# manoskary/analysisgnn

Measured on AMD Instinct MI355X. Metric: subgraph-nodes/sec fwd+bwd, HybridGNN L=3 H=256, higher is better.
Workload: dtype f32; 1 GPU; C2 (sampled, the batch a training step sees): HybridGNN L=3 H=256 out=128, 21 task heads, 32 neighbour-sampled subgraphs x (500 target notes + [5,5] hops) per GPU, per-hop counts passed (every layer trimmed); 16335 notes, 104099 edges per GPU; train step = fwd + objective (wloss) + bwd + allreduce + clip + AdamW, CSR rebuilt every step; hipGraph replay; workload_id=c2s, per_gpu_subgraphs=32, objective=wloss, parallelism=dp1, allreduce=none (one rank)

## Files before the change

analysisgnn_amd/_lib.py:

```python
from __future__ import annotations

import ctypes as C
import os
from typing import Optional, Sequence

import torch

from . import resident

_HERE = os.path.dirname(os.path.abspath(__file__))
LIB_PATH = os.path.join(_HERE, "libagnn_hip.so")
MAX_SEG = 32

SPMM_MEAN, SPMM_SKIP_SELF, SPMM_ACCUM = 1, 2, 4
INT32_MAX = 2 ** 31 - 1


class AgnnError(RuntimeError):
    pass


class CooSeg(C.Structure):
    _fields_ = [("row", C.c_void_p), ("col", C.c_void_p), ("etype", C.c_void_p),
                ("etype_code", C.c_int64), ("n_edges", C.c_int64), ("n_rows", C.c_int64)]
# ... 171 lines not shown
    "agnn_norm_act_fwd_f32": (C.c_int, [C.c_void_p, C.c_int64, C.c_void_p, C.c_void_p, C.c_int32, C.c_int64, C.c_int32, C.c_float, C.c_float,
                                        C.c_uint32, C.c_void_p, C.c_uint32, C.c_void_p, C.c_int64, C.c_void_p, C.c_void_p, C.c_void_p,
                                        C.c_void_p]),
    "agnn_norm_act_bwd_f32": (C.c_int, [C.c_void_p, C.c_int64, C.c_void_p, C.c_void_p, C.c_int32, C.c_int64, C.c_int32, C.c_float, C.c_float,
                                        C.c_uint32, C.c_void_p, C.c_uint32, C.c_void_p, C.c_int64, C.c_void_p, C.c_void_p, C.c_void_p,
                                        C.c_int64, C.c_void_p, C.c_void_p, C.c_void_p, C.c_size_t, C.c_void_p]),
    "agnn_norm_act_colsum_batch_f32": (C.c_int, [C.c_int32, C.POINTER(ColsumItem), C.c_void_p]),
    "agnn_skip_act_workspace_bytes": (C.c_size_t, []),
    "agnn_skip_act_fwd_f32": (C.c_int, [C.c_void_p, C.c_int64, C.c_void_p, C.c_int64, C.c_void_p, C.c_int64, C.c_int32, C.c_float, C.c_uint32,
                                        C.c_void_p, C.c_uint32, C.c_void_p, C.c_int64, C.c_void_p, C.c_void_p]),
    "agnn_skip_act_bwd_f32": (C.c_int, [C.c_void_p, C.c_int64, C.c_void_p, C.c_int64, C.c_void_p, C.c_int64, C.c_int32, C.c_float, C.c_uint32,
                                        C.c_void_p, C.c_uint32, C.c_void_p, C.c_int64, C.c_void_p, C.c_int64, C.c_void_p, C.c_int64, C.c_void_p,
                                        C.c_void_p, C.c_size_t, C.c_void_p]),
    "agnn_norm_act_colsum_f32": (C.c_int, [C.c_void_p, C.c_size_t, C.c_int64, C.c_int32, C.c_void_p, C.c_void_p, C.c_void_p]),
    "agnn_wgrad_workspace_bytes": (C.c_size_t, [C.c_int64, C.c_int32, C.c_int32]),
    "agnn_wgrad_f32": (C.c_int, [C.c_void_p, C.c_int64, C.c_void_p, C.c_int64, C.c_int64, C.c_int32, C.c_int32, C.c_void_p,
                                 C.c_int64, C.c_void_p, C.c_void_p, C.c_size_t, C.c_void_p]),
    "agnn_pack_f32": (C.c_int, [C.c_int32, C.POINTER(PackItem), C.c_void_p]),
    "agnn_gather_f32": (C.c_int, [C.c_int32, C.POINTER(GatherItem), C.c_void_p]),
    "agnn_debug_stamp": (C.c_int, [C.c_void_p, C.c_void_p]),
    "agnn_gproj_fwd_f32": (C.c_int, [C.c_void_p, C.c_int64, C.c_void_p, C.c_void_p, C.c_void_p, C.c_int32, C.c_int32, C.c_int32,
                                     C.c_int64, C.c_void_p, C.c_int64, C.c_void_p]),
    "agnn_gproj_workspace_bytes": (C.c_size_t, [C.c_int64, C.c_int32, C.c_int32, C.c_int32]),
    "agnn_gproj_bwd_f32": (C.c_int, [C.c_void_p, C.c_int64, C.c_void_p, C.c_int64, C.c_void_p, C.c_void_p, C.c_int32, C.c_int32,
                                     C.c_int32, C.c_int32, C.c_int64, C.c_void_p, C.c_int64, C.c_void_p, C.c_void_p, C.c_void_p,
                                     C.c_size_t, C.c_void_p]),
    "agnn_spmm_self_grad_f32": (C.c_int, [C.c_void_p, C.c_int64, C.c_int64, C.c_int32, C.c_void_p, C.c_int64, C.c_int64, C.c_int32,
                                          C.c_void_p, C.c_int64, C.c_int32, C.c_void_p]),
    "agnn_embed_cat_fwd_f32": (C.c_int, [C.c_void_p, C.c_int64, C.c_int32, C.c_int64, C.c_int32, C.POINTER(C.c_void_p),
                                         C.POINTER(C.c_void_p), C.POINTER(C.c_int32), C.c_int32, C.c_void_p, C.c_int64, C.c_void_p]),
    "agnn_embed_workspace_bytes": (C.c_size_t, [C.c_int32, C.POINTER(C.c_int32), C.c_int32]),
    "agnn_embed_cat_bwd_f32": (C.c_int, [C.c_void_p, C.c_int64, C.c_int32, C.c_int64, C.c_int32, C.POINTER(C.c_void_p),
                                         C.POINTER(C.c_int32), C.c_int32, C.c_void_p, C.c_void_p, C.c_size_t, C.c_void_p]),
    "agnn_train_loss_workspace_bytes": (C.c_size_t, []),
    "agnn_train_loss_f32": (C.c_int, [C.c_void_p, C.c_int64, C.c_void_p, C.c_int32, C.c_void_p, C.c_int64, C.c_float, C.c_int64,
                                      C.c_void_p, C.c_int64, C.c_int32, C.c_float, C.c_void_p, C.c_float, C.c_void_p, C.c_void_p,
                                      C.c_void_p, C.c_void_p, C.c_void_p, C.c_void_p, C.c_void_p, C.c_void_p, C.c_size_t,
                                      C.c_void_p]),
    "agnn_train_loss_final_f32": (C.c_int, [C.c_void_p, C.c_int64, C.c_void_p, C.c_int32, C.c_void_p, C.c_int64, C.c_float, C.c_int64,
                                            C.c_void_p, C.c_int64, C.c_int32, C.c_float, C.c_void_p, C.c_float, C.c_void_p, C.c_void_p,
                                            C.c_void_p, C.c_void_p, C.c_void_p, C.c_void_p, C.c_void_p, C.c_void_p, C.c_int64, C.c_void_p,
                                            C.c_size_t, C.c_void_p]),
    "agnn_train_loss_bwd_f32": (C.c_int, [C.c_void_p, C.c_int64, C.c_void_p, C.c_int32, C.c_int64, C.c_int32, C.c_void_p, C.c_void_p,
                                          C.c_void_p, C.c_int64, C.c_void_p, C.c_int64, C.c_int32, C.c_float, C.c_void_p, C.c_int64,
                                          C.c_void_p]),
    "agnn_adamw_workspace_bytes": (C.c_size_t, []),
    "agnn_adamw_f32": (C.c_int, [C.c_void_p, C.c_void_p, C.c_void_p, C.c_void_p, C.c_int64, C.c_float, C.c_float, C.c_float,
                                 C.c_float, C.c_float, C.c_float, C.c_void_p, C.c_void_p, C.c_int32, C.c_void_p, C.c_size_t,
                                 C.c_void_p]),
    "agnn_lr_schedule_at": (C.c_double, [C.POINTER(LrSchedule), C.c_int64]),
    "agnn_adamw_sched_workspace_bytes": (C.c_size_t, []),
    "agnn_adamw_sched_f32": (C.c_int, [C.c_void_p, C.c_void_p, C.c_void_p, C.c_void_p, C.c_int64, C.POINTER(LrSchedule), C.c_float,
                                       C.c_float, C.c_float, C.c_float, C.c_float, C.c_void_p, C.c_void_p, C.c_void_p, C.c_void_p,
                                       C.c_int32, C.c_void_p, C.c_size_t, C.c_void_p]),
    "agnn_multitask_ce_f32": (C.c_int, [C.c_void_p, C.c_int64, C.c_void_p, C.c_int32, C.c_void_p, C.c_int64, C.c_float,
                                        C.c_int64, C.c_void_p, C.c_void_p, C.c_void_p, C.c_void_p, C.c_void_p]),
    "agnn_multitask_ce_scale_f32": (C.c_int, [C.c_void_p, C.c_int64, C.c_void_p, C.c_int32, C.c_int64, C.c_int32, C.c_void_p,
                                              C.c_void_p, C.c_int64, C.c_void_p]),
    "agnn_kd_workspace_bytes": (C.c_size_t, [C.c_int64, C.c_int32]),
    "agnn_multitask_kd_f32": (C.c_int, [C.c_void_p, C.c_int64, C.c_void_p, C.c_int64, C.c_void_p, C.c_void_p, C.c_int32, C.c_int64,
                                        C.c_int32, C.c_float, C.c_float, C.c_void_p, C.c_int64, C.c_void_p, C.c_void_p, C.c_void_p,
                                        C.c_size_t, C.c_void_p]),
    "agnn_ewc_workspace_bytes": (C.c_size_t, []),
    "agnn_ewc_f32": (C.c_int, [C.c_void_p, C.c_void_p, C.c_void_p, C.c_int64, C.c_float, C.c_void_p, C.c_void_p, C.c_void_p,
                               C.c_size_t, C.c_void_p]),
    "agnn_fisher_accum_f32": (C.c_int, [C.c_void_p, C.c_int64, C.c_float, C.c_void_p, C.c_void_p]),
# ... 99 lines not shown
```

analysisgnn_amd/csrc/embed.hip:

```cpp
#include <cstdlib>

#include "agnn_common.h"

namespace {

constexpr int kMaxTab = AGNN_EMBED_MAX_TABLES;
constexpr int kSlices = 128;

struct EmbFwd {
  const float* x;
  int64_t ld_x;
  int32_t in_x, n_tab, dim;
  int64_t n_rows;
  const int64_t* idx[kMaxTab];
  const float* tab[kMaxTab];
  int32_t vocab[kMaxTab];
  float* out;
  int64_t ld_out;
};

__global__ __launch_bounds__(256) void k_embed_cat_fwd(EmbFwd a) {
  const int64_t total = a.n_rows * a.ld_out;
  for (int64_t e = static_cast<int64_t>(blockIdx.x) * 256 + threadIdx.x; e < total; e += static_cast<int64_t>(gridDim.x) * 256) {
    const int64_t row = e / a.ld_out;
// ... 152 lines not shown
  if (n_tab <= 0 || n_tab > kMaxTab) return fail(AGNN_EINVAL, "embed_bwd: n_tab=%d not in [1,%d]", n_tab, kMaxTab);
  if (n_rows < 0 || col0 < 0 || dim <= 0 || (dim & 1)) return fail(AGNN_EINVAL, "embed_bwd: bad sizes n_rows=%lld col0=%d dim=%d (dim must be even)", (long long)n_rows, col0, dim);
  if (!dout || !idx || !vocab || !dtables || !workspace) return fail(AGNN_EINVAL, "embed_bwd: null argument");
  if (ld_dout < static_cast<int64_t>(col0) + static_cast<int64_t>(n_tab) * dim) return fail(AGNN_EINVAL, "embed_bwd: ld_dout smaller than the row");
  if (reinterpret_cast<uintptr_t>(dtables) & 7u) return fail(AGNN_EALIGN, "embed_bwd: dtables must be 8-byte aligned");
  const size_t need = agnn_embed_workspace_bytes(n_tab, vocab, dim);
  if (need == 0 || workspace_bytes < need) return fail(AGNN_ENOMEM, "embed_bwd: workspace %zu < %zu bytes", workspace_bytes, need);
  EmbBwd a{};
  a.dout = dout; a.ld_dout = ld_dout; a.col0 = col0; a.n_tab = n_tab; a.dim = dim; a.dim_pad = dim; a.n_rows = n_rows;
  int vt = 0;
  for (int t = 0; t < n_tab; ++t) {
    if (!idx[t] || vocab[t] <= 0) return fail(AGNN_EINVAL, "embed_bwd: table %d: null index pointer or empty table", t);
    a.idx[t] = idx[t];
    a.vbase[t] = vt;
    vt += vocab[t];
  }
  a.vbase[n_tab] = vt;
  a.v_total = vt; a.v_pad = vt;
  a.slab = reinterpret_cast<float*>((reinterpret_cast<uintptr_t>(workspace) + 255) & ~uintptr_t{255});
  hipStream_t s = static_cast<hipStream_t>(stream_);
  const int ncg = (n_tab * dim + 63) / 64;
  if (static_cast<int64_t>(vt) * dim <= kEmbLdsFloats && ncg <= 4) {
    if (ncg == 1) hipLaunchKernelGGL(k_embed_bwd_rows<1>, dim3(kSlices), dim3(256), 0, s, a);
    else if (ncg == 2) hipLaunchKernelGGL(k_embed_bwd_rows<2>, dim3(kSlices), dim3(256), 0, s, a);
    else if (ncg == 3) hipLaunchKernelGGL(k_embed_bwd_rows<3>, dim3(kSlices), dim3(256), 0, s, a);
    else hipLaunchKernelGGL(k_embed_bwd_rows<4>, dim3(kSlices), dim3(256), 0, s, a);
    if (int rc = check_launch("embed_bwd(rows)")) return rc;
  } else {
    hipLaunchKernelGGL(k_embed_bwd, dim3(vt, kSlices), dim3(256), 0, s, a);
    if (int rc = check_launch("embed_bwd")) return rc;
  }
  return launch_slab_reduce(a.slab, nullptr, kSlices * 4, vt, dim, vt, dim, dtables, dim, nullptr, s);
}
```

analysisgnn_amd/embedding.py:

```python
from __future__ import annotations

import torch
import torch.nn.functional as F

import ctypes as C
from typing import Sequence

from . import _lib
from .linear import all_steal, weight_grad, wgrad_stream

MAX_ROWS = 256


class _SmallEmbedding(torch.autograd.Function):
    @staticmethod
    def forward(ctx, idx, weight):
        ctx.save_for_backward(idx)
        ctx.rows = weight.shape[0]
        ctx.leaf = weight.is_leaf
        ctx.weight_ref = weight if weight.is_leaf else None
        return F.embedding(idx, weight)

    @staticmethod
    def backward(ctx, dy):
        (idx,) = ctx.saved_tensors
        V = ctx.rows
        Vp = V + (V & 1)
        with wgrad_stream(dy.device, dy, idx, active=ctx.leaf and all_steal((ctx.weight_ref,)), kind="embed"):
            flat_idx = idx.reshape(-1)
            onehot = (flat_idx.unsqueeze(1) == torch.arange(Vp, device=idx.device)).to(dy.dtype)
            dy2 = dy.reshape(-1, dy.shape[-1]).contiguous()
            dw, _ = weight_grad(onehot, dy2, False)
            dw = dw[:V]
        return None, dw


def embedding(idx: torch.Tensor, weight: torch.Tensor) -> torch.Tensor:
    if weight.is_cuda and weight.requires_grad and torch.is_grad_enabled() and weight.shape[0] <= MAX_ROWS:
        return _SmallEmbedding.apply(idx, weight)
    return F.embedding(idx, weight)

# ... 26 lines not shown
        ctx.meta = (n, in_x, n_tab, dim, [int(t.shape[0]) for t in tabs], all(t.is_leaf for t in tabs))
        ctx.tab_refs = [t for t in tabs if t.is_leaf]
        return out[:, :width]

    @staticmethod
    def backward(ctx, dout):
        idc = ctx.saved_tensors
        n, in_x, n_tab, dim, vocabs, leaf = ctx.meta
        lib = _lib.load()
        dev = dout.device
        if dout.stride(1) != 1 or dout.dtype != torch.float32:
            dout = dout.float().contiguous()
        with wgrad_stream(dev, dout, *idc, active=leaf and all_steal(ctx.tab_refs), kind="embed"):
            vocab = (C.c_int32 * n_tab)(*vocabs)
            dtab = torch.empty((sum(vocabs), dim), dtype=torch.float32, device=dev)
            nws = int(lib.agnn_embed_workspace_bytes(n_tab, vocab, dim))
            ws = torch.empty(nws, dtype=torch.uint8, device=dev)
            _lib.check(lib.agnn_embed_cat_bwd_f32(dout.data_ptr(), dout.stride(0), in_x, n, n_tab, _ptr_array(idc), vocab, dim,
                                                  dtab.data_ptr(), ws.data_ptr(), nws, _lib.stream_ptr(dev)), "agnn_embed_cat_bwd_f32")
            grads = list(torch.split(dtab, vocabs, dim=0))
        return (None, None, *([None] * n_tab), *grads)


def embed_cat(x: torch.Tensor, idxs: Sequence[torch.Tensor], tables: Sequence[torch.Tensor]) -> torch.Tensor:
    n_tab = len(tables)
    fits = (x.is_cuda and x.dim() == 2 and 1 <= n_tab <= MAX_TABLES and len(idxs) == n_tab and not x.requires_grad
            and all(t.dim() == 2 and t.shape[1] == tables[0].shape[1] and t.dtype == torch.float32 for t in tables)
            and tables[0].shape[1] % 2 == 0 and all(i.dim() == 1 and i.shape[0] == x.shape[0] for i in idxs))
    if not fits:
        return torch.cat([x] + [embedding(i, t) for i, t in zip(idxs, tables)], dim=-1)
    r = _EmbedCat.apply(x, n_tab, *idxs, *tables)
    r._agnn_grad_cols = (int(x.shape[1]), int(r.shape[1]))
    return r
```

analysisgnn_amd/fused.py:

```python
from __future__ import annotations

import itertools
from typing import Optional

import torch
import torch.nn as nn
import torch.nn.functional as F

from . import _lib, resident
from .linear import ColsumItem, all_steal, defer, deferring, grad_slot_groups, leaf_refs, slot_group

PRE_RELU, POST_RELU = 1, 2
ENABLED = True
_CALL_IDS = itertools.count(1)


def rng_state(device) -> torch.Tensor:
    return resident.value(device, ("dropout counter",), lambda: torch.tensor([int(torch.initial_seed()) & 0x7FFFFFFFFFFFFFFF, 0],
                                                                             dtype=torch.int64, device=device))


def advance_rng(device) -> None:
    rng_state(device)[1:2].add_(1)

# ... 138 lines not shown
            raise _lib.AgnnError("norm_act: precomputed results stand for a plain LayerNorm on the kernel path")
        if not (torch.is_grad_enabled() and (x.requires_grad or ln.weight.requires_grad or ln.bias.requires_grad)):
            return pre[0]
        return _NormAct.apply(x, ln.weight, ln.bias, ln.eps, 0.0, 0, next(_CALL_IDS) & 0xFFFFFFFF, 0, False, None, pre)
    if not usable:
        y = F.relu(x) if pre_relu else x
        y = ln(y)
        y = F.relu(y) if post_relu else y
        return F.dropout(y, p, training)
    x2 = x.reshape(-1, H)
    flags = (PRE_RELU if pre_relu else 0) | (POST_RELU if post_relu else 0)
    y = _NormAct.apply(x2, ln.weight, ln.bias, ln.eps, p if training else 0.0, flags, next(_CALL_IDS) & 0xFFFFFFFF)
    return y.view(x.shape)


def grouped_norm_act(x: torch.Tensor, gamma: torch.Tensor, beta: torch.Tensor, eps: float, pre_relu: bool = False, pre=None) -> torch.Tensor:
    N, G, H = x.shape
    W = G * H
    gl = H // 4
    ok = (ENABLED and x.is_cuda and x.dtype == torch.float32 and H % 4 == 0 and 256 % H == 0 and (gl & (gl - 1)) == 0 and W <= 2048)
    if not ok:
        if pre is not None:
            raise _lib.AgnnError("grouped_norm_act: precomputed results need the kernel path")
        y = F.relu(x) if pre_relu else x
        return F.layer_norm(y, (H,), None, None, eps) * gamma + beta
    view_only = all(t.is_leaf or getattr(t, "_agnn_wgrad_deferrable", False) for t in (gamma, beta))
    y = _NormAct.apply(x.reshape(N, W), gamma.reshape(W), beta.reshape(W), eps, 0.0, PRE_RELU if pre_relu else 0,
                       next(_CALL_IDS) & 0xFFFFFFFF, H, view_only, leaf_refs(gamma, beta), pre, (slot_group(gamma), slot_group(beta)))
    return y.view(N, G, H)


class FusedSequential(nn.Sequential):

    def forward(self, x, pre=None):
        mods = list(self)
        i = 0
        if pre is not None:
            if not mods or not isinstance(mods[0], nn.LayerNorm) or (len(mods) > 1 and isinstance(mods[1], (nn.ReLU, nn.Dropout))):
                raise _lib.AgnnError("FusedSequential: precomputed results need a leading plain LayerNorm")
            x = norm_act(x, mods[0], pre=pre)
            i = 1
        while i < len(mods):
            m = mods[i]
            nxt = mods[i + 1] if i + 1 < len(mods) else None
            nn2 = mods[i + 2] if i + 2 < len(mods) else None
            if isinstance(m, nn.ReLU) and isinstance(nxt, nn.LayerNorm):
                p, used = (nn2.p, 3) if isinstance(nn2, nn.Dropout) else (0.0, 2)
                x = norm_act(x, nxt, pre_relu=True, p=p, training=self.training)
                i += used
            elif isinstance(m, nn.LayerNorm):
                post = isinstance(nxt, nn.ReLU)
                d = mods[i + 1 + int(post)] if i + 1 + int(post) < len(mods) else None
                p = d.p if isinstance(d, nn.Dropout) else 0.0
                x = norm_act(x, m, post_relu=post, p=p, training=self.training)
                i += 1 + int(post) + int(isinstance(d, nn.Dropout))
            else:
                x = m(x)
                i += 1
        return x
```

analysisgnn_amd/models.py:

```python
from __future__ import annotations

from typing import Dict, Optional

import torch
import torch.nn as nn
import torch.nn.functional as F

from . import _lib, ops
from .encoders import HybridGNN, MetricalGNN
from .fused import FusedSequential, _al16, advance_rng
from .embedding import embed_cat
from .heads import CrossTaskTransformer, fused_head_logits, fused_logit_fusion
from .linear import Linear
from .graph import SegSpec, build_csr


JOIN_FUSED = True


def _onset_index(n: int, onset_edges: torch.Tensor, batch_size: int, index):
    et = ("note", "onset", "note")
    if index is not None and et in index.bwd and index.bwd[et].n_rows >= n:
        return index.bwd[et], index.fwd[et]
    fwd, bwd = build_csr([SegSpec(onset_edges[0], onset_edges[1], n_rows=max(n, batch_size)),
                          SegSpec(onset_edges[1], onset_edges[0], n_rows=max(n, batch_size))])
    return fwd, bwd


class _PoolCat(torch.autograd.Function):

    @staticmethod
    def forward(ctx, x, fwd, bwd, n_pool, col_limit, gamma, beta, eps, box):
        dev = x.device
        lib = _lib.load()
        n, H = x.shape
        u = torch.empty((n, 2 * H), dtype=torch.float32, device=dev)
        y = torch.empty((n, 2 * H), dtype=torch.float32, device=dev)
        mean = torch.empty((n,), dtype=torch.float32, device=dev)
        rstd = torch.empty((n,), dtype=torch.float32, device=dev)
        inv_cnt = torch.empty((n,), dtype=torch.float32, device=dev)
        rel = _lib.make_rels([dict(src=None, rowptr=fwd.rowptr.data_ptr(), col=fwd.col.data_ptr(), ld_src=0)])
        _lib.check(lib.agnn_pool_cat_norm_f32(rel, x.data_ptr(), x.stride(0), n, n_pool, H, min(int(col_limit), _lib.INT32_MAX), gamma.data_ptr(),
                                              beta.data_ptr(), float(eps), u.data_ptr(), u.stride(0), y.data_ptr(), y.stride(0), mean.data_ptr(),
                                              rstd.data_ptr(), inv_cnt.data_ptr(), _lib.stream_ptr(dev)), "agnn_pool_cat_norm_f32")
        box.extend([y, mean, rstd])
        ctx.bwd, ctx.n_pool = bwd, n_pool
        ctx.save_for_backward(inv_cnt)
        return u

# ... 79 lines not shown
            self.cross_task_transformer = CrossTaskTransformer(o // 2, num_heads=4, dropout=dropout)
            self.fusion_layers = nn.ModuleDict({t: nn.Linear(o // 2, c) for t, c in task_dict.items()})
        self.rnn, self.rnn_norm, self.rnn_mlp = nn.Identity(), nn.Identity(), nn.Identity()

    def adjacent_parameter_groups(self):
        mods = list(self.clf_dict.values())
        groups = [[m[0].weight for m in mods], [m[0].bias for m in mods], [m[2].weight for m in mods],
                  [m[2].bias for m in mods], [m[3].weight for m in mods], [m[3].bias for m in mods]]
        rnn = getattr(self.encoder, "rnn", None)
        if isinstance(rnn, nn.GRU) and rnn.bidirectional:
            for layer in range(rnn.num_layers):
                for n in ("weight_ih", "weight_hh", "bias_ih", "bias_hh"):
                    groups.append([getattr(rnn, f"{n}_l{layer}"), getattr(rnn, f"{n}_l{layer}_reverse")])
        return groups

    split_backward = False

    def late_parameters(self):
        return [*self.project_dict.parameters(), *self.pitch_embedding.parameters(), *self.key_embedding.parameters()]

    def finish_backward(self) -> None:
        cut, self._cut = getattr(self, "_cut", None), None
        if cut:
            live = [(h, leaf.grad) for h, leaf in cut if leaf.grad is not None]
            if live:
                torch.autograd.backward([h for h, _ in live], [g for _, g in live])

    @torch._dynamo.disable
    def encode(self, pitch_spelling, key_signature, x_dict, edge_index_dict, batch_dict, batch_size,
               neighbor_mask_node, neighbor_mask_edge):
        if self.training:
            advance_rng(x_dict["note"].device)
        z_dict = dict(x_dict)
        z_dict["note"] = embed_cat(z_dict["note"], [pitch_spelling, key_signature],
                                   [self.pitch_embedding.weight, self.key_embedding.weight])
        for k, z in z_dict.items():
            if k != "note" and z.is_cuda and z.dim() == 2 and (z.shape[1] & 1) and z.stride(1) == 1 and z.stride(0) == z.shape[1] and z.shape[0] > 0:
                z_dict[k] = F.pad(z, (0, 1))[:, :z.shape[1]]
        h_dict = {k: self.project_dict[k](z_dict[k]) for k in self.project_dict.keys()}
        self._cut = None
        if self.split_backward and torch.is_grad_enabled():
            self._cut = []
            for k, hk in list(h_dict.items()):
                if hk.requires_grad:
                    leaf = hk.detach().requires_grad_(True)
                    self._cut.append((hk, leaf))
                    h_dict[k] = leaf
        x = self.encoder(x_dict=h_dict, edge_index_dict=edge_index_dict, batch_dict=batch_dict,
                         batch_size=batch_size, neighbor_mask_node=neighbor_mask_node,
                         neighbor_mask_edge=neighbor_mask_edge, return_edge_index=False, edge_attr_dict=None)
        index = getattr(getattr(self.encoder, "gnn", None), "last_index", None)
        onset = edge_index_dict[("note", "onset", "note")]
        joined = pool_cat_norm(x, onset, batch_size, self.project_enc[0], index) if JOIN_FUSED and x.is_cuda else None
        if joined is not None:
            return self.project_enc(joined[0], pre=joined[1])
        return self.project_enc(onset_pool(x, onset, batch_size, index))

    @torch._dynamo.disable
    def forward_clf(self, x, tasks=None):
        logits, offs, tasks = self.forward_clf_fused(x, tasks)
        return {t: logits[:, offs[i]:offs[i + 1]] for i, t in enumerate(tasks)}

    @torch._dynamo.disable
    def forward_clf_fused(self, x, tasks=None):
        tasks = list(self.clf_dict.keys() if tasks is None else tasks)
        logits, offs = fused_head_logits(self.clf_dict, x, tasks)
        if self.logit_fusion:
            logits = fused_logit_fusion(self.clf_proj_layers, self.cross_task_transformer, self.fusion_layers, logits, offs,
                                        tasks, self.training)
        return logits, offs, tasks

    def forward(self, pitch_spelling, key_signature, x_dict, edge_index_dict, batch_dict, batch_size,
# ... 7 lines not shown
```

include/agnn.h:

```cpp
#ifndef AGNN_H_
#define AGNN_H_

#include <stddef.h>
#include <stdint.h>

#ifdef __cplusplus
extern "C" {
#endif

typedef void* agnn_stream_t;

#define AGNN_OK        0
#define AGNN_EINVAL  (-22)
#define AGNN_EALIGN  (-14)
#define AGNN_ENOMEM  (-12)
#define AGNN_ERUNTIME (-5)

#define AGNN_MAX_SEG 32

const char* agnn_last_error(void);
int agnn_version(void);

typedef struct {
  const int64_t* row;
// ... 221 lines not shown
  int32_t c0, c1;
} agnn_grad_dst_t;
typedef struct {
  const float* dy;
  const float* x;
  int64_t ld_dy, ld_x, n;
  int32_t out_f, in_f;
  int32_t n_dw, n_db;
  agnn_grad_dst_t dw[AGNN_PACK_MAX_SRC];
  float* db[AGNN_PACK_MAX_SRC];
} agnn_grad_item_t;
size_t agnn_grad_epilogue_workspace_bytes(int32_t n_items, const agnn_grad_item_t* items );
int agnn_grad_epilogue_f32(int32_t n_items, const agnn_grad_item_t* items , int32_t n_sums,
                           const agnn_colsum_item_t* sums , void* workspace, size_t workspace_bytes, agnn_stream_t stream);

#define AGNN_GATHER_MAX_ITEMS 128
typedef struct {
  float* dst;
  const float* src;
  int64_t n;
} agnn_gather_item_t;
int agnn_gather_f32(int32_t n_items, const agnn_gather_item_t* items , agnn_stream_t stream);

int agnn_debug_stamp(uint64_t* slot , agnn_stream_t stream);

#define AGNN_EMBED_MAX_TABLES 4
int agnn_embed_cat_fwd_f32(const float* x, int64_t ld_x, int32_t in_x, int64_t n_rows, int32_t n_tab,
                           const int64_t* const* idx, const float* const* tables, const int32_t* vocab, int32_t dim,
                           float* out, int64_t ld_out, agnn_stream_t stream);
size_t agnn_embed_workspace_bytes(int32_t n_tab, const int32_t* vocab, int32_t dim);
int agnn_embed_cat_bwd_f32(const float* dout, int64_t ld_dout, int32_t col0, int64_t n_rows, int32_t n_tab,
                           const int64_t* const* idx, const int32_t* vocab, int32_t dim, float* dtables,
                           void* workspace, size_t workspace_bytes, agnn_stream_t stream);

int agnn_heads_fwd_f32(const float* x, int64_t ld_x, int64_t n_rows, int32_t in_f, int32_t hidden, int32_t T, const float* w1,
                       const float* b1, const float* gamma, const float* beta, float eps, const float* w2, const float* b2,
                       const int32_t* offs_dev, const int32_t* offs_host, float* z, float* y, int64_t ld_h, float* mean,
                       float* rstd, float* logits, int64_t ld_o, agnn_stream_t stream);

int agnn_gproj_fwd_f32(const float* a, int64_t ld_a, const float* w, const float* b, const int32_t* seg_off,
                       int32_t n_groups, int32_t K, int32_t n_tiles32, int64_t n_rows, float* out, int64_t ld_out,
                       agnn_stream_t stream);
size_t agnn_gproj_workspace_bytes(int64_t n_rows, int32_t sum_c, int32_t K, int32_t n_tiles32);
int agnn_gproj_bwd_f32(const float* dout, int64_t ld_dout, const float* a, int64_t ld_a, const float* w,
                       const int32_t* seg_off, int32_t n_groups, int32_t K, int32_t n_tiles32, int32_t sum_c,
                       int64_t n_rows, float* da, int64_t ld_da, float* dw, float* db, void* workspace,
                       size_t workspace_bytes, agnn_stream_t stream);

int agnn_multitask_ce_f32(const float* logits, int64_t ld, const int32_t* seg_off, int32_t n_tasks,
                          const int64_t* labels, int64_t n_rows, float label_smoothing,
                          int64_t ignore_index, float* row_loss, float* dlogits, float* loss, float* inv_count,
                          agnn_stream_t stream);
int agnn_multitask_ce_scale_f32(const float* dlogits, int64_t ld, const int32_t* seg_off, int32_t n_tasks,
                                int64_t n_rows, int32_t n_cols, const float* scale, float* out, int64_t ld_out,
                                agnn_stream_t stream);

size_t agnn_train_loss_workspace_bytes(void);
int agnn_train_loss_f32(const float* logits, int64_t ld, const int32_t* seg_off, int32_t n_tasks, const int64_t* labels,
                        int64_t n_rows, float label_smoothing, int64_t ignore_index, const float* feat, int64_t ld_feat,
                        int32_t feat_cols, float lambda_feat, const float* task_param, float ce_scale, float* row_loss,
                        float* dlogits, float* loss, float* inv_count, float* total, float* wscale, float* dparam,
                        void* workspace, size_t workspace_bytes, agnn_stream_t stream);
int agnn_train_loss_final_f32(const float* logits, int64_t ld, const int32_t* seg_off, int32_t n_tasks, const int64_t* labels,
                              int64_t n_rows, float label_smoothing, int64_t ignore_index, const float* feat, int64_t ld_feat,
                              int32_t feat_cols, float lambda_feat, const float* task_param, float ce_scale, float* row_loss,
                              float* dlogits, float* loss, float* inv_count, float* total, float* wscale, float* dparam,
// ... 104 lines not shown
```

Measured before the change: 5.758 million subgraph-nodes/s.

## Pre-project embedding tables through first note Linear instead of concatenating

Replaces the embed_cat followed by the first Linear of the note projection MLP with a fused path. The table rows are multiplied by the matching slice of the weight once (at most 256 rows), and each node's output becomes a small dense GEMM over the raw features plus lookups of the pre-projected table rows. The backward scatters dy into per-row table sums held in LDS, then forms the table gradients and the table part of dW from those sums. This avoids materialising the concatenated input and running a full-width GEMM over the embedding columns, at the cost of new custom kernels, f64 accumulation in the table projection, and a changed order of float summation.

```diff
diff --git a/analysisgnn_amd/_lib.py b/analysisgnn_amd/_lib.py
--- a/analysisgnn_amd/_lib.py
+++ b/analysisgnn_amd/_lib.py
@@ -227,6 +227,13 @@
     "agnn_embed_workspace_bytes": (C.c_size_t, [C.c_int32, C.POINTER(C.c_int32), C.c_int32]),
     "agnn_embed_cat_bwd_f32": (C.c_int, [C.c_void_p, C.c_int64, C.c_int32, C.c_int64, C.c_int32, C.POINTER(C.c_void_p),
                                          C.POINTER(C.c_int32), C.c_int32, C.c_void_p, C.c_void_p, C.c_size_t, C.c_void_p]),
+    "agnn_embed_proj_workspace_bytes": (C.c_size_t, [C.c_int64, C.c_int32, C.c_int32, C.POINTER(C.c_int32), C.c_int32, C.c_int32]),
+    "agnn_embed_proj_fwd_f32": (C.c_int, [C.c_void_p, C.c_int64, C.c_int32, C.c_int64, C.c_int32, C.POINTER(C.c_void_p),
+                                          C.POINTER(C.c_void_p), C.POINTER(C.c_int32), C.c_int32, C.c_void_p, C.c_int64, C.c_void_p,
+                                          C.c_int32, C.c_void_p, C.c_size_t, C.c_void_p, C.c_int64, C.c_void_p, C.c_int64, C.c_void_p]),
+    "agnn_embed_proj_bwd_f32": (C.c_int, [C.c_void_p, C.c_int64, C.c_int64, C.c_int32, C.c_int32, C.c_int32, C.POINTER(C.c_void_p),
+                                          C.POINTER(C.c_void_p), C.POINTER(C.c_int32), C.c_int32, C.c_void_p, C.c_int64,
+                                          C.POINTER(C.c_void_p), C.c_void_p, C.c_int64, C.c_void_p, C.c_void_p, C.c_size_t, C.c_void_p]),
     "agnn_train_loss_workspace_bytes": (C.c_size_t, []),
     "agnn_train_loss_f32": (C.c_int, [C.c_void_p, C.c_int64, C.c_void_p, C.c_int32, C.c_void_p, C.c_int64, C.c_float, C.c_int64,
                                       C.c_void_p, C.c_int64, C.c_int32, C.c_float, C.c_void_p, C.c_float, C.c_void_p, C.c_void_p,
diff --git a/analysisgnn_amd/csrc/embed.hip b/analysisgnn_amd/csrc/embed.hip
--- a/analysisgnn_amd/csrc/embed.hip
+++ b/analysisgnn_amd/csrc/embed.hip
@@ -208,3 +208,398 @@
   }
   return launch_slab_reduce(a.slab, nullptr, kSlices * 4, vt, dim, vt, dim, dtables, dim, nullptr, s);
 }
+
+namespace {
+
+constexpr int kProjMaxRows = 256;
+constexpr int kProjMaxInX = 64;
+constexpr int kProjLdsBytes = 64 * 1024;
+constexpr int kProjMaxSlabs = 128;
+
+struct ProjTab {
+  const int64_t* idx[kMaxTab];
+  const float* tab[kMaxTab];
+  int32_t vbase[kMaxTab + 1];
+  int32_t n_tab, dim;
+};
+
+__global__ __launch_bounds__(256) void k_embed_proj_tables(ProjTab p, const float* __restrict__ W, int64_t ld_w, int in_x, int H,
+                                                           float* __restrict__ T) {
+  extern __shared__ float s_w[];
+  const int ncol = p.n_tab * p.dim;
+  float* s_e = s_w + 8 * (ncol + 1);
+  const int h0 = blockIdx.x * 8;
+  const int v0 = blockIdx.y * 32;
+  const int vt = p.vbase[p.n_tab];
+  for (int e = threadIdx.x; e < 8 * ncol; e += 256) {
+    const int h = e / ncol, c = e - h * ncol;
+    s_w[h * (ncol + 1) + c] = W[(h0 + h) * ld_w + in_x + c];
+  }
+  for (int e = threadIdx.x; e < 32 * p.dim; e += 256) {
+    const int vl = e / p.dim, d = e - vl * p.dim;
+    const int vg = v0 + vl < vt ? v0 + vl : vt - 1;
+    int t = 0;
+    while (t + 1 < p.n_tab && vg >= p.vbase[t + 1]) ++t;
+    s_e[vl * (p.dim + 1) + d] = p.tab[t][static_cast<int64_t>(vg - p.vbase[t]) * p.dim + d];
+  }
+  __syncthreads();
+  const int h = threadIdx.x & 7, vl = threadIdx.x >> 3;
+  const int vg = v0 + vl;
+  if (vg >= vt) return;
+  int t = 0;
+  while (t + 1 < p.n_tab && vg >= p.vbase[t + 1]) ++t;
+  const float* er = s_e + vl * (p.dim + 1);
+  const float* wr = s_w + h * (ncol + 1) + t * p.dim;
+  double acc = 0.0;
+  for (int d = 0; d < p.dim; ++d) acc = fma(static_cast<double>(er[d]), static_cast<double>(wr[d]), acc);
+  T[static_cast<int64_t>(vg) * H + h0 + h] = static_cast<float>(acc);
+}
+
+struct ProjFwd {
+  ProjTab tb;
+  const float* x;
+  int64_t ld_x, n_rows, ld_y, ld_w, ld_xpad;
+  const float* W;
+  const float* bias;
+  const float* T;
+  float* y;
+  float* xpad;
+  int32_t in_x, H;
+};
+
+template <int CS>
+__global__ __launch_bounds__(256) void k_embed_proj_fwd(ProjFwd a) {
+  constexpr int LPR = CS / 4;
+  constexpr int RPW = 64 / LPR;
+  constexpr int XJ = kProjMaxInX / LPR;
+  extern __shared__ __align__(16) float s_fwd[];
+  const int vt = a.tb.vbase[a.tb.n_tab];
+  float* s_t = s_fwd;
+  constexpr int WS = CS + 4;
+  float* s_wx = s_fwd + vt * CS;
+  const int c0 = blockIdx.y * CS;
+  for (int e = threadIdx.x; e < vt * CS; e += 256) {
+    const int v = e / CS, c = e - v * CS;
+    s_t[e] = a.T[static_cast<int64_t>(v) * a.H + c0 + c];
+  }
+  for (int e = threadIdx.x; e < a.in_x * CS; e += 256) {
+    const int c = e / a.in_x, k = e - c * a.in_x;
+    s_wx[k * WS + c] = a.W[(c0 + c) * a.ld_w + k];
+  }
+  __syncthreads();
+  const int lane = threadIdx.x & 63;
+  const int wave = threadIdx.x >> 6;
+  const int sub = lane / LPR, li = lane - sub * LPR;
+  const int col = li * 4;
+  const float4 b4 = *reinterpret_cast<const float4*>(a.bias + c0 + col);
+  const int64_t stride = static_cast<int64_t>(gridDim.x) * 4 * RPW;
+  const bool pad_writer = a.xpad != nullptr && blockIdx.y == 0;
+  int64_t r = (static_cast<int64_t>(blockIdx.x) * 4 + wave) * RPW + sub;
+  const int64_t last = a.n_rows - 1;
+  int id[kMaxTab];
+  float xv[XJ];
+  auto fetch = [&](int64_t row) {
+    const int64_t rr = row < last ? row : last;
+#pragma unroll
+    for (int t = 0; t < kMaxTab; ++t) {
+      const int tt = t < a.tb.n_tab ? t : 0;
+      const int64_t v = a.tb.idx[tt][rr];
+      const int vn = a.tb.vbase[tt + 1] - a.tb.vbase[tt];
+      id[t] = a.tb.vbase[tt] + static_cast<int>(v < 0 ? 0 : (v >= vn ? vn - 1 : v));
+    }
+#pragma unroll
+    for (int j = 0; j < XJ; ++j) {
+      const int k = li + j * LPR;
+      xv[j] = a.in_x > 0 ? a.x[rr * a.ld_x + (k < a.in_x ? k : a.in_x - 1)] : 0.f;
+    }
+  };
+  const int64_t r_end = ((a.n_rows + RPW - 1) / RPW) * RPW;
+  if (r < r_end) fetch(r);
+  for (; r < r_end; r += stride) {
+    int idc[kMaxTab];
+    float xc[XJ];
+#pragma unroll
+    for (int t = 0; t < kMaxTab; ++t) idc[t] = id[t];
+#pragma unroll
+    for (int j = 0; j < XJ; ++j) xc[j] = xv[j];
+    const int64_t nxt = r + stride;
+    fetch(nxt < r_end ? nxt : r);
+    float4 acc = b4;
+#pragma unroll
+    for (int j = 0; j < XJ; ++j) {
+      int kn = a.in_x - j * LPR;
+      kn = kn < 0 ? 0 : (kn > LPR ? LPR : kn);
+      for (int kk = 0; kk < kn; ++kk) {
+        const float xk = __shfl(xc[j], sub * LPR + kk, 64);
+        const float4 w = *reinterpret_cast<const float4*>(s_wx + (j * LPR + kk) * WS + col);
+        acc.x = fmaf(xk, w.x, acc.x);
+        acc.y = fmaf(xk, w.y, acc.y);
+        acc.z = fmaf(xk, w.z, acc.z);
+        acc.w = fmaf(xk, w.w, acc.w);
+      }
+    }
+#pragma unroll
+    for (int t = 0; t < kMaxTab; ++t) {
+      if (t < a.tb.n_tab) {
+        const float4 tv = *reinterpret_cast<const float4*>(s_t + idc[t] * CS + col);
+        acc.x += tv.x; acc.y += tv.y; acc.z += tv.z; acc.w += tv.w;
+      }
+    }
+    if (r < a.n_rows) {
+      *reinterpret_cast<float4*>(a.y + r * a.ld_y + c0 + col) = acc;
+      if (pad_writer) {
+#pragma unroll
+        for (int j = 0; j < XJ; ++j) {
+          const int k = li + j * LPR;
+          if (k < a.ld_xpad) a.xpad[r * a.ld_xpad + k] = k < a.in_x ? xc[j] : 0.f;
+        }
+      }
+    }
+  }
+}
+
+struct ProjBwd {
+  ProjTab tb;
+  const float* dy;
+  int64_t ld_dy, n_rows;
+  int32_t H, waves;
+  float* slab;
+};
+
+__global__ __launch_bounds__(256) void k_embed_proj_bwd_rows(ProjBwd a) {
+  extern __shared__ float s_mem[];
+  const int lane = threadIdx.x & 63;
+  const int wave = __builtin_amdgcn_readfirstlane(threadIdx.x >> 6);
+  const int vt = a.tb.vbase[a.tb.n_tab];
+  const int img = vt * 64;
+  float* acc = s_mem + wave * img;
+  for (int e = lane; e < img; e += 64) acc[e] = 0.f;
+  const int part = blockIdx.x * a.waves + wave;
+  const int64_t per = (a.n_rows + static_cast<int64_t>(gridDim.x) * a.waves - 1) / (static_cast<int64_t>(gridDim.x) * a.waves);
+  int64_t r0 = part * per;
+  int64_t r1 = r0 + per;
+  if (r1 > a.n_rows) r1 = a.n_rows;
+  if (r0 > r1) r0 = r1;
+  const int c = blockIdx.y * 64 + lane;
+  __builtin_amdgcn_fence(__ATOMIC_RELEASE, "wavefront");
+  __builtin_amdgcn_wave_barrier();
+  constexpr int RB = 8;
+  for (int64_t base = r0; base < r1; base += RB) {
+    float val[RB];
+    int id[RB][kMaxTab];
+#pragma unroll
+    for (int u = 0; u < RB; ++u) {
+      const int64_t r = base + u < r1 ? base + u : r1 - 1;
+      val[u] = base + u < r1 ? a.dy[r * a.ld_dy + c] : 0.f;
+#pragma unroll
+      for (int t = 0; t < kMaxTab; ++t) {
+        const int tt = t < a.tb.n_tab ? t : 0;
+        const int64_t v = a.tb.idx[tt][r];
+        const int vn = a.tb.vbase[tt + 1] - a.tb.vbase[tt];
+        id[u][t] = a.tb.vbase[tt] + static_cast<int>(v < 0 ? 0 : (v >= vn ? vn - 1 : v));
+      }
+    }
+#pragma unroll
+    for (int u = 0; u < RB; ++u)
+#pragma unroll
+      for (int t = 0; t < kMaxTab; ++t)
+        if (t < a.tb.n_tab) acc[id[u][t] * 64 + lane] += val[u];
+  }
+  __syncthreads();
+  float* dst = a.slab + static_cast<int64_t>(blockIdx.x) * vt * a.H + blockIdx.y * 64;
+  for (int e = threadIdx.x; e < img; e += blockDim.x) {
+    float s = s_mem[e];
+    for (int w = 1; w < a.waves; ++w) s += s_mem[w * img + e];
+    dst[static_cast<int64_t>(e >> 6) * a.H + (e & 63)] = s;
+  }
+}
+
+struct ProjOut {
+  ProjTab tb;
+  const float* G;
+  const float* W;
+  int64_t ld_w, ld_dw;
+  int32_t in_x, H;
+  float* dtab[kMaxTab];
+  float* dW;
+  float* db;
+};
+
+__global__ __launch_bounds__(256) void k_embed_proj_bwd_out(ProjOut a) {
+  __shared__ float s_g[kProjMaxRows * 8];
+  __shared__ float s_p[4][64];
+  const int vt = a.tb.vbase[a.tb.n_tab];
+  const int hb = a.H >> 3;
+  if (static_cast<int>(blockIdx.x) < hb) {
+    const int h0 = blockIdx.x * 8;
+    for (int e = threadIdx.x; e < vt * 8; e += 256) s_g[e] = a.G[static_cast<int64_t>(e >> 3) * a.H + h0 + (e & 7)];
+    __syncthreads();
+    const int ncol = a.tb.n_tab * a.tb.dim;
+    for (int e = threadIdx.x; e < 8 * ncol; e += 256) {
+      const int h = e / ncol, c = e - h * ncol;
+      const int t = c / a.tb.dim, d = c - t * a.tb.dim;
+      const int vb = a.tb.vbase[t], vn = a.tb.vbase[t + 1] - vb;
+      const float* ep = a.tb.tab[t] + d;
+      float acc = 0.f;
+#pragma unroll 4
+      for (int v = 0; v < vn; ++v) acc = fmaf(s_g[(vb + v) * 8 + h], ep[static_cast<int64_t>(v) * a.tb.dim], acc);
+      a.dW[(h0 + h) * a.ld_dw + a.in_x + c] = acc;
+    }
+    if (a.db) {
+      int vn = a.tb.vbase[1];
+      while (vn > 1) {
+        const int half = (vn + 1) >> 1;
+        __syncthreads();
+        for (int e = threadIdx.x; e < (vn - half) * 8; e += 256) s_g[e] += s_g[half * 8 + e];
+        vn = half;
+      }
+      __syncthreads();
+      if (threadIdx.x < 8) a.db[h0 + threadIdx.x] = s_g[threadIdx.x];
+    }
+    return;
+  }
+  const int vg = blockIdx.x - hb;
+  int t = 0;
+  while (t + 1 < a.tb.n_tab && vg >= a.tb.vbase[t + 1]) ++t;
+  for (int e = threadIdx.x; e < a.H; e += 256) s_g[e] = a.G[static_cast<int64_t>(vg) * a.H + e];
+  __syncthreads();
+  const int lane = threadIdx.x & 63, wave = threadIdx.x >> 6;
+  const int hq = a.H >> 2;
+  float* out = a.dtab[t] + static_cast<int64_t>(vg - a.tb.vbase[t]) * a.tb.dim;
+  for (int d0 = 0; d0 < a.tb.dim; d0 += 64) {
+    const int d = d0 + lane;
+    const int dd = d < a.tb.dim ? d : a.tb.dim - 1;
+    const float* wp = a.W + a.in_x + t * a.tb.dim + dd;
+    float acc = 0.f;
+#pragma unroll 8
+    for (int h = wave * hq; h < (wave + 1) * hq; ++h) acc = fmaf(s_g[h], wp[h * a.ld_w], acc);
+    s_p[wave][lane] = acc;
+    __syncthreads();
+    if (wave == 0 && d < a.tb.dim) out[d] = ((s_p[0][lane] + s_p[1][lane]) + s_p[2][lane]) + s_p[3][lane];
+    __syncthreads();
+  }
+}
+
+struct ProjShape {
+  int vt, cs, waves, slabs;
+  size_t fwd_lds, bwd_lds, tab_lds;
+};
+
+const char* proj_shape(int64_t n_rows, int32_t in_x, int32_t n_tab, const int32_t* vocab, int32_t dim, int32_t H, ProjShape* o) {
+  if (n_tab < 1 || n_tab > kMaxTab) return "n_tab not in [1, 4]";
+  if (n_rows < 0 || in_x < 0 || in_x > kProjMaxInX || dim <= 0 || (dim & 1) || H <= 0 || (H & 63)) return "bad sizes (in_x <= 64, dim even, H a multiple of 64)";
+  if (H > kProjMaxRows * 8) return "H too large";
+  if (!vocab) return "null argument";
+  int64_t vt = 0;
+  for (int t = 0; t < n_tab; ++t) {
+    if (vocab[t] <= 0) return "empty table";
+    vt += vocab[t];
+  }
+  if (vt > kProjMaxRows) return "more than 256 table rows in total";
+  o->vt = static_cast<int>(vt);
+  o->cs = (H % 128 == 0) ? 128 : 64;
+  auto lds = [&](int cs) { return (static_cast<size_t>(vt) * cs + static_cast<size_t>(in_x) * (cs + 4)) * sizeof(float); };
+  o->fwd_lds = lds(o->cs);
+  if (o->fwd_lds > static_cast<size_t>(kProjLdsBytes) && o->cs == 128) {
+    o->cs = 64;
+    o->fwd_lds = lds(64);
+  }
+  if (o->fwd_lds > static_cast<size_t>(kProjLdsBytes)) return "tables and feature weights do not fit the LDS ((rows + in_x) * 256 B > 64 KB, about)";
+  o->tab_lds = (static_cast<size_t>(8) * (static_cast<size_t>(n_tab) * dim + 1) + static_cast<size_t>(32) * (dim + 1)) * sizeof(float);
+  if (o->tab_lds > static_cast<size_t>(kProjLdsBytes)) return "table width too large";
+  const size_t image = static_cast<size_t>(vt) * 64 * sizeof(float);
+  int waves = static_cast<int>(kProjLdsBytes / image);
+  o->waves = waves > 4 ? 4 : waves;
+  int64_t slabs = (n_rows + o->waves * 16 - 1) / (o->waves * 16);
+  o->slabs = static_cast<int>(slabs < 1 ? 1 : (slabs > kProjMaxSlabs ? kProjMaxSlabs : slabs));
+  o->bwd_lds = image * o->waves;
+  return nullptr;
+}
+
+int proj_tab(ProjTab* p, int32_t n_tab, const int64_t* const* idx, const float* const* tables, const int32_t* vocab, int32_t dim) {
+  using namespace agnn;
+  if (!idx || !tables) return fail(AGNN_EINVAL, "embed_proj: null argument");
+  p->n_tab = n_tab; p->dim = dim;
+  int vt = 0;
+  for (int t = 0; t < n_tab; ++t) {
+    if (!idx[t] || !tables[t]) return fail(AGNN_EINVAL, "embed_proj: table %d: null pointer", t);
+    if (reinterpret_cast<uintptr_t>(tables[t]) & 7u) return fail(AGNN_EALIGN, "embed_proj: table %d must be 8-byte aligned", t);
+    p->idx[t] = idx[t]; p->tab[t] = tables[t]; p->vbase[t] = vt;
+    vt += vocab[t];
+  }
+  for (int t = n_tab; t <= kMaxTab; ++t) p->vbase[t] = vt;
+  return AGNN_OK;
+}
+
+}
+
+extern "C" size_t agnn_embed_proj_workspace_bytes(int64_t n_rows, int32_t in_x, int32_t n_tab, const int32_t* vocab, int32_t dim, int32_t H) {
+  ProjShape sh{};
+  if (proj_shape(n_rows, in_x, n_tab, vocab, dim, H, &sh)) return 0;
+  return (static_cast<size_t>(sh.slabs) + 1) * sh.vt * static_cast<size_t>(H) * sizeof(float) + 256;
+}
+
+extern "C" int agnn_embed_proj_fwd_f32(const float* x, int64_t ld_x, int32_t in_x, int64_t n_rows, int32_t n_tab,
+                                       const int64_t* const* idx, const float* const* tables, const int32_t* vocab, int32_t dim,
+                                       const float* W, int64_t ld_w, const float* bias, int32_t H, void* workspace,
+                                       size_t workspace_bytes, float* y, int64_t ld_y, float* x_pad, int64_t ld_xpad,
+                                       agnn_stream_t stream_) {
+  using namespace agnn;
+  ProjShape sh{};
+  if (const char* why = proj_shape(n_rows, in_x, n_tab, vocab, dim, H, &sh)) return fail(AGNN_EINVAL, "embed_proj_fwd: %s", why);
+  if (ld_w < static_cast<int64_t>(in_x) + static_cast<int64_t>(n_tab) * dim || ld_y < H || (in_x > 0 && ld_x < in_x))
+    return fail(AGNN_EINVAL, "embed_proj_fwd: leading dimension smaller than the row");
+  if (x_pad && (ld_xpad < in_x || ld_xpad > kProjMaxInX)) return fail(AGNN_EINVAL, "embed_proj_fwd: ld_xpad=%lld not in [in_x, 64]", (long long)ld_xpad);
+  if (n_rows == 0) return AGNN_OK;
+  if (!W || !bias || !workspace || !y || (in_x > 0 && !x)) return fail(AGNN_EINVAL, "embed_proj_fwd: null argument");
+  if (!aligned16(y) || (ld_y & 3) || !aligned16(bias)) return fail(AGNN_EALIGN, "embed_proj_fwd: y (and its row stride) and bias must be 16-byte aligned");
+  const size_t need = static_cast<size_t>(sh.vt) * H * sizeof(float) + 256;
+  if (workspace_bytes < need) return fail(AGNN_ENOMEM, "embed_proj_fwd: workspace %zu < %zu bytes", workspace_bytes, need);
+  ProjFwd a{};
+  if (int rc = proj_tab(&a.tb, n_tab, idx, tables, vocab, dim)) return rc;
+  float* T = reinterpret_cast<float*>((reinterpret_cast<uintptr_t>(workspace) + 255) & ~uintptr_t{255});
+  hipStream_t s = static_cast<hipStream_t>(stream_);
+  hipLaunchKernelGGL(k_embed_proj_tables, dim3(H / 8, (sh.vt + 31) / 32), dim3(256), sh.tab_lds, s, a.tb, W, ld_w, in_x, H, T);
+  if (int rc = check_launch("embed_proj_fwd(tables)")) return rc;
+  a.x = x; a.ld_x = ld_x; a.n_rows = n_rows; a.ld_y = ld_y; a.ld_w = ld_w; a.ld_xpad = ld_xpad; a.W = W; a.bias = bias; a.T = T;
+  a.y = y; a.xpad = x_pad; a.in_x = in_x; a.H = H;
+  const int rpw = 64 / (sh.cs / 4);
+  const int slices = H / sh.cs;
+  int64_t blocks = (n_rows + 4 * rpw - 1) / (4 * rpw);
+  const int64_t cap = 512 / slices > 0 ? 512 / slices : 1;
+  if (blocks > cap) blocks = cap;
+  if (sh.cs == 128) hipLaunchKernelGGL(k_embed_proj_fwd<128>, dim3(static_cast<unsigned>(blocks), slices), dim3(256), sh.fwd_lds, s, a);
+  else hipLaunchKernelGGL(k_embed_proj_fwd<64>, dim3(static_cast<unsigned>(blocks), slices), dim3(256), sh.fwd_lds, s, a);
+  return check_launch("embed_proj_fwd");
+}
+
+extern "C" int agnn_embed_proj_bwd_f32(const float* dy, int64_t ld_dy, int64_t n_rows, int32_t H, int32_t in_x, int32_t n_tab,
+                                       const int64_t* const* idx, const float* const* tables, const int32_t* vocab, int32_t dim,
+                                       const float* W, int64_t ld_w, float* const* dtables, float* dW, int64_t ld_dw, float* db,
+                                       void* workspace, size_t workspace_bytes, agnn_stream_t stream_) {
+  using namespace agnn;
+  ProjShape sh{};
+  if (const char* why = proj_shape(n_rows, in_x, n_tab, vocab, dim, H, &sh)) return fail(AGNN_EINVAL, "embed_proj_bwd: %s", why);
+  const int64_t width = static_cast<int64_t>(in_x) + static_cast<int64_t>(n_tab) * dim;
+  if (ld_w < width || ld_dw < width || ld_dy < H) return fail(AGNN_EINVAL, "embed_proj_bwd: leading dimension smaller than the row");
+  if (!dy || !W || !dtables || !dW || !workspace) return fail(AGNN_EINVAL, "embed_proj_bwd: null argument");
+  const size_t need = agnn_embed_proj_workspace_bytes(n_rows, in_x, n_tab, vocab, dim, H);
+  if (workspace_bytes < need) return fail(AGNN_ENOMEM, "embed_proj_bwd: workspace %zu < %zu bytes", workspace_bytes, need);
+  ProjOut o{};
+  if (int rc = proj_tab(&o.tb, n_tab, idx, tables, vocab, dim)) return rc;
+  for (int t = 0; t < n_tab; ++t) {
+    if (!dtables[t]) return fail(AGNN_EINVAL, "embed_proj_bwd: table %d: null gradient pointer", t);
+    o.dtab[t] = dtables[t];
+  }
+  float* G = reinterpret_cast<float*>((reinterpret_cast<uintptr_t>(workspace) + 255) & ~uintptr_t{255});
+  hipStream_t s = static_cast<hipStream_t>(stream_);
+  ProjBwd a{};
+  a.tb = o.tb; a.dy = dy; a.ld_dy = ld_dy; a.n_rows = n_rows; a.H = H; a.waves = sh.waves;
+  a.slab = G + static_cast<size_t>(sh.vt) * H;
+  hipLaunchKernelGGL(k_embed_proj_bwd_rows, dim3(sh.slabs, H / 64), dim3(64 * sh.waves), sh.bwd_lds, s, a);
+  if (int rc = check_launch("embed_proj_bwd(rows)")) return rc;
+  if (int rc = launch_slab_reduce(a.slab, nullptr, sh.slabs, sh.vt, H, sh.vt, H, G, H, nullptr, s)) return rc;
+  o.G = G; o.W = W; o.ld_w = ld_w; o.ld_dw = ld_dw; o.in_x = in_x; o.H = H; o.dW = dW; o.db = db;
+  hipLaunchKernelGGL(k_embed_proj_bwd_out, dim3(H / 8 + sh.vt), dim3(256), 0, s, o);
+  return check_launch("embed_proj_bwd(out)");
+}
diff --git a/analysisgnn_amd/embedding.py b/analysisgnn_amd/embedding.py
--- a/analysisgnn_amd/embedding.py
+++ b/analysisgnn_amd/embedding.py
@@ -7,6 +7,7 @@
 from typing import Sequence
 
 from . import _lib
+from . import linear as _linear
 from .linear import all_steal, weight_grad, wgrad_stream
 
 MAX_ROWS = 256
@@ -99,3 +100,102 @@
     r = _EmbedCat.apply(x, n_tab, *idxs, *tables)
     r._agnn_grad_cols = (int(x.shape[1]), int(r.shape[1]))
     return r
+
+
+PROJ_MAX_IN_X = 64
+PROJ_TABLES_IN_PLACE = False
+
+
+def _proj_vocab(tables):
+    return (C.c_int32 * len(tables))(*[int(t.shape[0]) for t in tables])
+
+
+def embed_project_fits(x, idxs, tables, weight, bias) -> bool:
+    n_tab = len(tables)
+    if not (x.is_cuda and x.dim() == 2 and x.dtype == torch.float32 and x.stride(1) == 1 and not x.requires_grad and x.shape[0] > 0
+            and 1 <= n_tab <= MAX_TABLES and len(idxs) == n_tab and bias is not None and x.shape[1] <= PROJ_MAX_IN_X):
+        return False
+    dim = int(tables[0].shape[1]) if tables[0].dim() == 2 else 0
+    if not (dim > 0 and dim % 2 == 0 and all(t.dim() == 2 and t.shape[1] == dim and t.dtype == torch.float32 and t.is_cuda and t.is_contiguous()
+                                             and t.data_ptr() % 8 == 0 for t in tables)
+            and all(i.dim() == 1 and i.shape[0] == x.shape[0] and i.is_cuda and not i.is_floating_point() for i in idxs)):
+        return False
+    H = int(weight.shape[0])
+    if not (weight.dim() == 2 and weight.dtype == torch.float32 and weight.is_cuda and weight.is_contiguous() and weight.shape[1] == x.shape[1] + n_tab * dim
+            and H % 64 == 0 and bias.dtype == torch.float32 and bias.is_contiguous() and tuple(bias.shape) == (H,) and bias.data_ptr() % 16 == 0):
+        return False
+    return int(_lib.load().agnn_embed_proj_workspace_bytes(int(x.shape[0]), int(x.shape[1]), n_tab, _proj_vocab(tables), dim, H)) > 0
+
+
+class _EmbedProject(torch.autograd.Function):
+    @staticmethod
+    def forward(ctx, x, weight, bias, n_tab, *rest):
+        idxs, tabs = rest[:n_tab], rest[n_tab:]
+        lib = _lib.load()
+        dev = x.device
+        n, in_x = int(x.shape[0]), int(x.shape[1])
+        dim, H = int(tabs[0].shape[1]), int(weight.shape[0])
+        idc = [i if (i.dtype == torch.int64 and i.is_contiguous()) else i.long().contiguous() for i in idxs]
+        vocab = _proj_vocab(tabs)
+        want_grad = bool(ctx.needs_input_grad[1])
+        x_ok = in_x % 2 == 0 and x.stride(0) % 2 == 0 and x.data_ptr() % 8 == 0
+        xp = None
+        if want_grad and in_x > 0 and not x_ok:
+            xp = torch.empty((n, (in_x + 1) & ~1), dtype=torch.float32, device=dev)
+        y = torch.empty((n, H), dtype=torch.float32, device=dev)
+        nws = int(lib.agnn_embed_proj_workspace_bytes(n, in_x, n_tab, vocab, dim, H))
+        ws = torch.empty(nws, dtype=torch.uint8, device=dev)
+        _lib.check(lib.agnn_embed_proj_fwd_f32(x.data_ptr(), x.stride(0), in_x, n, n_tab, _ptr_array(idc), _ptr_array(tabs), vocab, dim,
+                                               weight.data_ptr(), weight.stride(0), bias.data_ptr(), H, ws.data_ptr(), nws, y.data_ptr(), H,
+                                               _lib.ptr(xp), (xp.shape[1] if xp is not None else 0), _lib.stream_ptr(dev)), "agnn_embed_proj_fwd_f32")
+        ctx.save_for_backward(weight, *tabs, *idc)
+        ctx.x_op = (xp[:, :in_x] if xp is not None else x) if in_x > 0 else None
+        ctx.meta = (n, in_x, n_tab, dim, H, nws)
+        ctx.refs = (weight, bias, *tabs) if all(t.is_leaf for t in (weight, bias, *tabs)) else None
+        ctx.set_materialize_grads(False)
+        return y
+
+    @staticmethod
+    def backward(ctx, dy):
+        n, in_x, n_tab, dim, H, nws = ctx.meta
+        none = (None,) * (4 + 2 * n_tab)
+        if dy is None:
+            return none
+        saved = ctx.saved_tensors
+        weight, tabs, idc = saved[0], saved[1:1 + n_tab], saved[1 + n_tab:]
+        lib = _lib.load()
+        dev = dy.device
+        if dy.stride(1) != 1 or dy.dtype != torch.float32 or dy.stride(0) % 2 or dy.data_ptr() % 8:
+            dy = dy.float().contiguous()
+        refs = ctx.refs
+        steals = refs is not None and all_steal(refs)
+        slots = _linear.grad_slots(refs if PROJ_TABLES_IN_PLACE else refs[:2]) if steals else None
+        if slots is not None:
+            dW, db, dtabs = slots[0], slots[1], (list(slots[2:]) or [torch.empty_like(t) for t in tabs])
+        else:
+            dW = torch.empty((H, in_x + n_tab * dim), dtype=torch.float32, device=dev)
+            db = torch.empty((H,), dtype=torch.float32, device=dev)
+            dtabs = [torch.empty_like(t) for t in tabs]
+        del slots
+        dW_k = dW.detach()
+        vocab = _proj_vocab(tabs)
+        with wgrad_stream(dev, dy, weight, dW_k, db, *dtabs, *idc, *tabs, active=steals, kind="embed"):
+            ws = torch.empty(nws, dtype=torch.uint8, device=dev)
+            _lib.check(lib.agnn_embed_proj_bwd_f32(dy.data_ptr(), dy.stride(0), n, H, in_x, n_tab, _ptr_array(idc), _ptr_array(tabs), vocab, dim,
+                                                   weight.data_ptr(), weight.stride(0), _ptr_array(dtabs), dW_k.data_ptr(), dW_k.stride(0),
+                                                   db.data_ptr(), ws.data_ptr(), nws, _lib.stream_ptr(dev)), "agnn_embed_proj_bwd_f32")
+        if in_x > 0:
+            xo = ctx.x_op
+            if steals and _linear.deferring(dy) and (in_x % 2 == 0 or xo.stride(0) > in_x):
+                xk = xo.as_strided((n, (in_x + 1) & ~1), (xo.stride(0), 1), xo.storage_offset()) if in_x & 1 else xo
+                _linear.defer(_linear.WgItem(dy, xk, False, None, None, dsts=[(0, in_x, dW_k[:, :in_x])], db_dsts=()), dev, here=True)
+            else:
+                with wgrad_stream(dev, dy, xo, dW_k, active=steals):
+                    dwx, _ = weight_grad(dy, xo, False)
+                    dW_k[:, :in_x].copy_(dwx)
+        return (None, dW, db, None, *([None] * n_tab), *dtabs)
+
+
+def embed_project(x: torch.Tensor, idxs: Sequence[torch.Tensor], tables: Sequence[torch.Tensor], weight: torch.Tensor,
+                  bias: torch.Tensor) -> torch.Tensor:
+    return _EmbedProject.apply(x, weight, bias, len(tables), *idxs, *tables)
diff --git a/analysisgnn_amd/fused.py b/analysisgnn_amd/fused.py
--- a/analysisgnn_amd/fused.py
+++ b/analysisgnn_amd/fused.py
@@ -194,9 +194,9 @@
 
 class FusedSequential(nn.Sequential):
 
-    def forward(self, x, pre=None):
+    def forward(self, x, pre=None, start=0):
         mods = list(self)
-        i = 0
+        i = int(start)
         if pre is not None:
             if not mods or not isinstance(mods[0], nn.LayerNorm) or (len(mods) > 1 and isinstance(mods[1], (nn.ReLU, nn.Dropout))):
                 raise _lib.AgnnError("FusedSequential: precomputed results need a leading plain LayerNorm")
diff --git a/analysisgnn_amd/models.py b/analysisgnn_amd/models.py
--- a/analysisgnn_amd/models.py
+++ b/analysisgnn_amd/models.py
@@ -9,12 +9,13 @@
 from . import _lib, ops
 from .encoders import HybridGNN, MetricalGNN
 from .fused import FusedSequential, _al16, advance_rng
-from .embedding import embed_cat
+from .embedding import embed_cat, embed_project, embed_project_fits
 from .heads import CrossTaskTransformer, fused_head_logits, fused_logit_fusion
 from .linear import Linear
 from .graph import SegSpec, build_csr
 
 
+INPUT_TABLES_PROJECTED = True
 JOIN_FUSED = True
 
 
@@ -160,12 +161,20 @@
         if self.training:
             advance_rng(x_dict["note"].device)
         z_dict = dict(x_dict)
-        z_dict["note"] = embed_cat(z_dict["note"], [pitch_spelling, key_signature],
-                                   [self.pitch_embedding.weight, self.key_embedding.weight])
+        tables = [self.pitch_embedding.weight, self.key_embedding.weight]
+        note_mlp = self.project_dict["note"] if "note" in self.project_dict else None
+        first = note_mlp[0] if isinstance(note_mlp, FusedSequential) and len(note_mlp) > 0 else None
+        y_note = None
+        if (INPUT_TABLES_PROJECTED and type(first) is Linear
+                and embed_project_fits(z_dict["note"], [pitch_spelling, key_signature], tables, first.weight, first.bias)):
+            y_note = embed_project(z_dict["note"], [pitch_spelling, key_signature], tables, first.weight, first.bias)
+        else:
+            z_dict["note"] = embed_cat(z_dict["note"], [pitch_spelling, key_signature], tables)
         for k, z in z_dict.items():
             if k != "note" and z.is_cuda and z.dim() == 2 and (z.shape[1] & 1) and z.stride(1) == 1 and z.stride(0) == z.shape[1] and z.shape[0] > 0:
                 z_dict[k] = F.pad(z, (0, 1))[:, :z.shape[1]]
-        h_dict = {k: self.project_dict[k](z_dict[k]) for k in self.project_dict.keys()}
+        h_dict = {k: (note_mlp(y_note, start=1) if (k == "note" and y_note is not None) else self.project_dict[k](z_dict[k]))
+                  for k in self.project_dict.keys()}
         self._cut = None
         if self.split_backward and torch.is_grad_enabled():
             self._cut = []
diff --git a/include/agnn.h b/include/agnn.h
--- a/include/agnn.h
+++ b/include/agnn.h
@@ -277,6 +277,16 @@
 int agnn_embed_cat_bwd_f32(const float* dout, int64_t ld_dout, int32_t col0, int64_t n_rows, int32_t n_tab,
                            const int64_t* const* idx, const int32_t* vocab, int32_t dim, float* dtables,
                            void* workspace, size_t workspace_bytes, agnn_stream_t stream);
+
+size_t agnn_embed_proj_workspace_bytes(int64_t n_rows, int32_t in_x, int32_t n_tab, const int32_t* vocab, int32_t dim, int32_t H);
+int agnn_embed_proj_fwd_f32(const float* x, int64_t ld_x, int32_t in_x, int64_t n_rows, int32_t n_tab,
+                            const int64_t* const* idx, const float* const* tables, const int32_t* vocab, int32_t dim,
+                            const float* W, int64_t ld_w, const float* bias, int32_t H, void* workspace, size_t workspace_bytes,
+                            float* y, int64_t ld_y, float* x_pad, int64_t ld_xpad, agnn_stream_t stream);
+int agnn_embed_proj_bwd_f32(const float* dy, int64_t ld_dy, int64_t n_rows, int32_t H, int32_t in_x, int32_t n_tab,
+                            const int64_t* const* idx, const float* const* tables, const int32_t* vocab, int32_t dim,
+                            const float* W, int64_t ld_w, float* const* dtables, float* dW, int64_t ld_dw, float* db,
+                            void* workspace, size_t workspace_bytes, agnn_stream_t stream);
 
 int agnn_heads_fwd_f32(const float* x, int64_t ld_x, int64_t n_rows, int32_t in_f, int32_t hidden, int32_t T, const float* w1,
                        const float* b1, const float* gamma, const float* beta, float eps, const float* w2, const float* b2,
```

Measured after the change: 5.742 million subgraph-nodes/s. About the same (-0.3%).
